# Renatovela-ctrl/dsp-audio-project

Measured on AMD Instinct MI355X. Metric: Msamples/sec SRC→6-biquad EQ→FFT chain at 1/2/4/8 MI355X; % HBM roofline, higher is better.
Workload: dtype f32 (IIR state/coefficients f64); 1 GPU; config 4: 32768 ch x 48000 @48kHz sharded over the GPUs: SRC L3/M2 K121 -> 6-biquad EQ @72kHz -> 4096-pt FFT |X| of centre segment; total_channels=32768, channels_per_gpu=32768, n_in=48000, n_out=72000, fs_in=48000, L=3, M=2, n_fft=4096, parallelism=channel-shard x1 (no collective), launch=hipGraph

## Files before the change

dsp-audio-project_amd/csrc/chain_tile.h:

```cpp
#pragma once
#include <algorithm>
#include <cmath>
#include <cstring>
#include <type_traits>

#include "cascade.h"

namespace dsp {


constexpr int kStream = 2;
constexpr int kSc1 = 16;
constexpr int kLS = 32;
constexpr int kS = 6;
constexpr int kD = 2 * kS;
constexpr int kNPMax = 32;
constexpr int kScanRow = 14;
constexpr int kScanPark = 928;
constexpr int kScanFloats = (kScanPark + 16) * 2;


typedef float f32x4 __attribute__((ext_vector_type(4)));
typedef float f32x2 __attribute__((ext_vector_type(2)));

__host__ __device__ constexpr int xpad(int g) { return g + 4 * (g >> 5); }

template <int L_, int M_, int TT_, int CR_>
struct TileGeo {
  static constexpr int L = L_, M = M_, TT = TT_, CR = CR_;
  static_assert((kLS * L) % M == 0, "32 input samples per sub-chunk must make whole outputs");
  static_assert(M % 2 == 0, "packed taps: windows of one branch share their x parity");
  static constexpr int TSUB = kLS * L / M;
  static constexpr int TILE = kWave * TSUB;
  static_assert(TSUB % 12 == 0 && TSUB <= kWave, "SRC in parts of 12; two float4 halves");
  static constexpr int NP = TT / 2 + 1;
  static_assert(NP <= kNPMax, "tap pairs");
  static constexpr int qi(int i) { return (i * M + CR) / L; }
  static constexpr int phi(int i) { return (i * M + CR) % L; }
  static constexpr int qs(int i) { return qi(i) & ~1; }
  static constexpr int W = qs(TSUB - 1) + 2 * NP;
  static constexpr int NWIN = (kLS * (kWave - 1) + W + 3) / 4 * 4;
  static constexpr int XF = xpad(NWIN + 4) + 4;
  static constexpr int RS = TSUB + 4;
  static constexpr int SF = (kWave / 2) * RS;
  static constexpr int CF = (kWave + 1) * kD * 2;
  static constexpr int LDSF0 = XF > SF ? (XF > CF ? XF : CF) : (SF > CF ? SF : CF);
  static constexpr int LDSF = LDSF0 > kScanFloats ? LDSF0 : kScanFloats;
  static_assert(L <= 4, "four branch slots per tap pair row");
  static_assert(qs(TSUB - 1) < W, "");
};

template <class GEO>
constexpr int branch_parity(int ph) {
  int a = -1;
  for (int i = 0; i < GEO::TSUB; ++i)
    if (GEO::phi(i) == ph) {
      const int ai = GEO::qi(i) & 1;
      if (a >= 0 && a != ai) return -2;
      a = ai;
    }
  return a;
}

constexpr int kGenTS = 32;
constexpr int kGenTile = kWave * kGenTS;
constexpr int kGenWaves = 4;
constexpr int kGenTT = 8;
constexpr int kGenClasses = 8;
constexpr int kGenClassStride = kGenTS * kGenTT + 4;
constexpr int kCtTaps = 10;
constexpr int kCtRow = 12;
constexpr int kCtClassStride = kGenTS * kCtRow + 4;

constexpr int kPpSlots = 16;
constexpr int kPpTapFloats = 1024;

struct TileTables {
  uint64_t key;
  double G[64][kD];
  float Gc[32][kD][2];
  double Q[kD][kD];
  double Dp[6][kS][4];
  double T[kD][kD];
  float TP[kNPMax][4][2];
  int32_t tsub, np, L, M, K, S;
  double cf[kS][4];
  double gain;
  float seq[kGenClasses][kGenTS][kGenTT];
  uint32_t adv[kGenClasses];
  int32_t classes, pad;
  alignas(16) float seqs[kGenClasses][kGenTS][kCtRow];
  float flush_thr;
  int32_t pad3[3];
  alignas(16) float tpw[kPpTapFloats];
  float pp_td;
  int32_t pp_np, pp_geo, pad4;
};

struct TileArgs {
  const float* x;
  float* y;
  float* z;
  const TileTables* tt;
  double* states;
  uint32_t* flags;
  uint32_t* err;
  int64_t B, n_in, ld_x, n_out, ld_y, ntiles, cq;
  int clip;
  uint32_t max_spins;
  const float* taps;
  int64_t c;
  int K, L, M, T, win;
};

__device__ __forceinline__ void fence() { asm volatile("" ::: "memory"); }

__device__ __forceinline__ int lane_id() {
  return (int)__builtin_amdgcn_mbcnt_hi(~0u, __builtin_amdgcn_mbcnt_lo(~0u, 0u));
}

template <int N, class T>
__device__ __forceinline__ void pin(T (&v)[N]) {
#pragma unroll
  for (int i = 0; i < N; ++i) asm volatile("" : "+v"(v[i]));
}

template <class PTR>
__device__ __forceinline__ void mac2(PTR M, double x0, double x1, double& a0, double& a1) {
  a0 = fma(M[0], x0, fma(M[1], x1, a0));
  a1 = fma(M[2], x0, fma(M[3], x1, a1));
}

__device__ __forceinline__ double shfl_up_f64(double v, int d) {
  const int src = ((int)threadIdx.x - d) << 2;
  const uint64_t u = __double_as_longlong(v);
  const uint32_t lo = __builtin_amdgcn_ds_bpermute(src, (int)(uint32_t)u);
  const uint32_t hi = __builtin_amdgcn_ds_bpermute(src, (int)(uint32_t)(u >> 32));
  return __longlong_as_double((long long)(((uint64_t)hi << 32) | lo));
}

__device__ __forceinline__ double shfl_f64(double v, int src) {
  const uint64_t u = __double_as_longlong(v);
  const uint32_t lo = __builtin_amdgcn_ds_bpermute(src << 2, (int)(uint32_t)u);
  const uint32_t hi = __builtin_amdgcn_ds_bpermute(src << 2, (int)(uint32_t)(u >> 32));
  return __longlong_as_double((long long)(((uint64_t)hi << 32) | lo));
}

__device__ __forceinline__ uint32_t load_flag(const uint32_t* p) {
  return __hip_atomic_load((const __attribute__((address_space(1))) uint32_t*)p,
                           __ATOMIC_RELAXED, __HIP_MEMORY_SCOPE_AGENT);
}
__device__ __forceinline__ void store_flag(uint32_t* p, uint32_t v) {
  __hip_atomic_store((__attribute__((address_space(1))) uint32_t*)p, v,
                     __ATOMIC_RELAXED, __HIP_MEMORY_SCOPE_AGENT);
}
__device__ __forceinline__ double load_state(const double* p) {
  return __hip_atomic_load((const __attribute__((address_space(1))) double*)p,
                           __ATOMIC_RELAXED, __HIP_MEMORY_SCOPE_AGENT);
}
__device__ __forceinline__ void store_state(double* p, double v) {
  __hip_atomic_store((__attribute__((address_space(1))) double*)p, v,
                     __ATOMIC_RELAXED, __HIP_MEMORY_SCOPE_AGENT);
}

typedef __attribute__((address_space(4))) const TileTables* tt_ptr;

template <class GEO>
constexpr bool dly_out(int i) { return GEO::phi(i) == 0; }
template <class GEO>
constexpr bool void_pair(int p, int ph) {
  const int a = branch_parity<GEO>(ph);
  if (a < 0) return true;
  for (int e = 0; e < 2; ++e) {
    const int u = 2 * p + e - a;
    if (u >= 0 && u < GEO::TT && ph + GEO::L * (GEO::TT - 1 - u) < 40 * GEO::L + 1) return false;
  }
  return true;
}
struct VoidPairs {
  bool v[kNPMax][4];
};
template <class GEO>
constexpr VoidPairs void_pairs() {
  VoidPairs t{};
  for (int p = 0; p < kNPMax; ++p)
    for (int ph = 0; ph < 4; ++ph) t.v[p][ph] = ph < GEO::L && p < GEO::NP && void_pair<GEO>(p, ph);
  return t;
}
template <class GEO>
constexpr int dly_slot() { return GEO::TT / 2 + (branch_parity<GEO>(0) > 0 ? 1 : 0); }

template <class GEO, int H0, int NH, bool DLY = false>
__device__ __forceinline__ void src_part(const float* xw, tt_ptr tt, float (&y)[GEO::TSUB]) {
  static constexpr VoidPairs kVoid = void_pairs<GEO>();
  constexpr int V0 = GEO::qs(H0) / 4 * 4;
  constexpr int V1 = GEO::qs(H0 + NH - 1) + 2 * GEO::NP;
  constexpr int NV = (V1 - V0 + 3) / 4 * 4;
  f32x2 w[NV / 2];
#pragma unroll
  for (int k = 0; k < NV / 4; ++k) {
    const f32x4 f = *reinterpret_cast<const f32x4*>(xw + xpad(V0 + 4 * k));
    w[2 * k] = f32x2{f.x, f.y};
    w[2 * k + 1] = f32x2{f.z, f.w};
  }
  f32x2 acc[NH];
#pragma unroll
  for (int i = 0; i < NH; ++i) acc[i] = f32x2{0.f, 0.f};
#pragma unroll
  for (int p = 0; p < GEO::NP; ++p) {
    tt_ptr tq = tt;
    asm volatile("" : "+s"(tq));
    f32x2 t[GEO::L];
#pragma unroll
    for (int ph = 0; ph < GEO::L; ++ph) t[ph] = f32x2{tq->TP[p][ph][0], tq->TP[p][ph][1]};
#pragma unroll
    for (int i = 0; i < NH; ++i)
      if (!(DLY && (dly_out<GEO>(H0 + i) || kVoid.v[p][GEO::phi(H0 + i)])))
        acc[i] = __builtin_elementwise_fma(t[GEO::phi(H0 + i)],
                                           w[(GEO::qs(H0 + i) - V0) / 2 + p], acc[i]);
  }
  float td = 0.f;
  if (DLY) {
    tt_ptr tq = tt;
    asm volatile("" : "+s"(tq));
    td = tq->TP[dly_slot<GEO>() / 2][0][dly_slot<GEO>() % 2];
  }
#pragma unroll
  for (int i = 0; i < NH; ++i) {
    if (DLY && dly_out<GEO>(H0 + i)) {
      const f32x2 xv = w[(GEO::qs(H0 + i) - V0) / 2 + dly_slot<GEO>() / 2];
      y[H0 + i] = td * (dly_slot<GEO>() % 2 ? xv.y : xv.x);
    } else {
      y[H0 + i] = acc[i].x + acc[i].y;
    }
  }
}

template <int TS>
struct StageBase {
  int b[3];
  __device__ __forceinline__ explicit StageBase(int lane) {
    if constexpr (TS == 32) {
      b[0] = 32 * (lane >> 3) + 4 * ((lane & 7) ^ ((lane >> 3) & 7));
    } else if constexpr (TS != 48) {
      static_assert(TS % 4 == 0, "staging rows of whole float4s");
      b[0] = lane;
    } else {
      const int a = (lane * 43) >> 9;
      const int r = lane - 12 * a;
      b[0] = 4 * lane + 4 * a;
      b[1] = b[0] + 4 * ((r + 8) >> 4);
      b[2] = b[0] + 4 * ((r + 12) >> 4);
    }
  }
  __device__ __forceinline__ int at(int k) const {
    if constexpr (TS == 32) return b[0] + 256 * k;
    else if constexpr (TS != 48) {
      const int g = 4 * (b[0] + kWave * k);
      return g + 4 * (g / TS);
    } else return b[k % 3] + 276 * k + (k >= 3 ? 4 : 0);
  }
};

template <int TS>
__device__ __forceinline__ void store_tile(float* lds, const float (&v)[TS], int lane,
                                           __amdgpu_buffer_rsrc_t rs) {
  constexpr int RS = TS == 32 ? 32 : TS + 4;
  constexpr int NF4 = (kWave / 2) * TS / 4;
  constexpr int NR = (NF4 + kWave - 1) / kWave;
  typedef unsigned int u32x4 __attribute__((ext_vector_type(4)));
  const StageBase<TS> sb(lane);
#pragma unroll
  for (int h = 0; h < 2; ++h) {
    fence();
    if ((lane >> 5) == h) {
      float* row = lds + (lane & 31) * RS;
      const int sw = TS == 32 ? (lane & 7) : 0;
#pragma unroll
      for (int k = 0; k < TS / 4; ++k)
        *reinterpret_cast<float4*>(row + 4 * (k ^ sw)) =
            make_float4(v[4 * k], v[4 * k + 1], v[4 * k + 2], v[4 * k + 3]);
    }
    fence();
#pragma unroll
    for (int k = 0; k < NR; ++k) {
      const int g = 4 * (lane + kWave * k);
      const bool past = NF4 % kWave && k == NR - 1 && lane + kWave * k >= NF4;
      const float4 f = *reinterpret_cast<const float4*>(lds + sb.at(k));
      u32x4 d;
      d.x = __float_as_uint(f.x);
      d.y = __float_as_uint(f.y);
      d.z = __float_as_uint(f.z);
      d.w = __float_as_uint(f.w);
      __builtin_amdgcn_raw_buffer_store_b128(d, rs, past ? 0x7ffffff0 : (h * (kWave / 2) * TS + g) * 4,
                                             0, kStream);
    }
  }
  fence();
}

__device__ __forceinline__ void tile_entry_state(const TileArgs& a, int64_t b, int64_t tile,
                                                 int lane, double (&m_in)[kD]) {
  if (lane == 0) {
    const int64_t prev = b * a.ntiles + tile - 1;
    uint32_t spins = 0;
    bool ok = true;
    while (load_flag(a.flags + prev) == 0u) {
      if (++spins > a.max_spins) {
        store_flag(a.err, 1u);
        ok = false;
        break;
      }
      __builtin_amdgcn_s_sleep(2);
    }
    fence();
#pragma unroll
    for (int d = 0; d < kD; ++d) m_in[d] = load_state(a.states + prev * kD + d);
    if (ok) store_flag(a.flags + prev, 0u);
  }
}

__host__ __device__ constexpr int staging_floats(int ts) { return (kWave / 2) * (ts + 4); }

__device__ __forceinline__ void pass1_basis(tt_ptr mt, const f32x2 (&e2)[kD], double (&v)[kD]);

template <int TS>
__device__ __forceinline__ void pass1_state(tt_ptr mt, const float (&y)[TS], double (&v)[kD]) {
  {
    f32x2 e2[kD];
#pragma unroll
    for (int d = 0; d < kD; ++d) e2[d] = f32x2{-0.f, -0.f};
#pragma unroll
    for (int j = 0; j < TS / 2; ++j) {
      tt_ptr tq = mt;
      asm volatile("" : "+s"(tq));
      const f32x2 u = f32x2{y[2 * j], y[2 * j + 1]};
#pragma unroll
      for (int d = 0; d < kD; ++d)
        e2[d] = __builtin_elementwise_fma(f32x2{tq->Gc[j][d][0], tq->Gc[j][d][1]}, u, e2[d]);
    }
    pin(e2);
    pass1_basis(mt, e2, v);
  }
}

template <int TS>
__device__ __forceinline__ void pass1_state_f64(tt_ptr mt, const float (&y)[TS], double (&v)[kD]) {
#pragma unroll
  for (int d = 0; d < kD; ++d) v[d] = 0.0;
#pragma unroll
  for (int i = 0; i < TS; ++i) {
    tt_ptr tq = mt;
    asm volatile("" : "+s"(tq));
    const double u = (double)y[i];
#pragma unroll
    for (int d = 0; d < kD; ++d) v[d] = fma(tq->G[i][d], u, v[d]);
  }
}

__device__ __forceinline__ void pass1_basis(tt_ptr mt, const f32x2 (&e2)[kD], double (&v)[kD]) {
  {
    f32x2 e[kS];
#pragma unroll
    for (int k = 0; k < kS; ++k)
      e[k] = f32x2{e2[2 * k].x + e2[2 * k].y, e2[2 * k + 1].x + e2[2 * k + 1].y};
    double ed[kD];
#pragma unroll
    for (int k = 0; k < kS; ++k) {
      ed[2 * k] = (double)e[k].x;
      ed[2 * k + 1] = (double)e[k].y;
    }
#pragma unroll
    for (int r = kD - 1; r >= 0; --r) {
      tt_ptr tq = mt;
      asm volatile("" : "+s"(tq));
      double acc = tq->Q[r][0] * ed[0];
#pragma unroll
      for (int c = 1; c <= r; ++c) acc = fma(tq->Q[r][c], ed[c], acc);
      v[r] = acc;
    }
  }
}

template <int TS, bool NANCLIP>
__device__ __forceinline__ void pass2_cascade(const TileArgs& a, tt_ptr mt, float (&y)[TS],
                                              const double (&m)[kD]) {
  double s1[kS], s2[kS];
#pragma unroll
  for (int r = 0; r < kD; ++r) {
    double acc = m[r];
#pragma unroll
    for (int cc = 0; cc < (r / 2) * 2; ++cc) acc = fma(mt->T[r][cc], m[cc], acc);
    if (r & 1) s2[r / 2] = acc;
    else s1[r / 2] = acc;
  }
  float lo = a.clip ? -1.f : -INFINITY, hi = a.clip ? 1.f : INFINITY;
  asm volatile("" : "+v"(lo), "+v"(hi));
  const float g32 = (float)mt->gain;
  {
    double pend[kS];
#pragma unroll
    for (int st = 0; st < TS + kS - 1; ++st) {
#pragma unroll
      for (int k = kS - 1; k >= 0; --k) {
        const int t = st - k;
        if (t < 0 || t >= TS) continue;
        const double u = k == 0 ? (double)y[t] : pend[k - 1];
        const double c1 = mt->cf[k][0], c2 = mt->cf[k][1], a1 = mt->cf[k][2], a2 = mt->cf[k][3];
        const double w = fma(-a2, s2[k], fma(-a1, s1[k], u));
        const double v2 = fma(c2, s2[k], fma(c1, s1[k], w));
        s2[k] = s1[k];
        s1[k] = w;
        if (k == kS - 1)
          y[t] = NANCLIP ? clip_f32((float)v2 * g32, lo, hi)
                         : __builtin_amdgcn_fmed3f((float)v2 * g32, lo, hi);
        else pend[k] = v2;
      }
    }
  }
}

template <int TS, bool P1F64 = false, class SUMS>
__device__ __forceinline__ void fix_outputs(const TileArgs& a, tt_ptr mt, int64_t b, int64_t z0,
                                            float (&y)[TS], double (&v)[kD], SUMS&& sums) {
  const __amdgpu_buffer_rsrc_t rz = __builtin_amdgcn_make_buffer_rsrc(
      a.z + b * a.ld_y, 0, (int)(a.n_out * 4), 0x00020000);
  const int off0 = (int)(z0 * 4);
  auto get = [&](int i) {
    return __uint_as_float(__builtin_amdgcn_raw_buffer_load_b32(rz, off0 + 4 * i, 0, 1));
  };
  auto put = [&](int i, float f) {
    __builtin_amdgcn_raw_buffer_store_b32(__float_as_uint(f), rz, off0 + 4 * i, 0, 0);
  };
#pragma unroll
  for (int i = 0; i < TS; ++i) put(i, y[i]);
  asm volatile("s_waitcnt vmcnt(0)" ::: "memory");
  bool any = false;
#pragma unroll 1
  for (int i = 0; i < TS; ++i) {
    float nf, fin, f = get(i);
    sums(i, nf, fin);
    any |= nf_fix(f, nf, fin);
    put(i, f);
  }
  asm volatile("s_waitcnt vmcnt(0)" ::: "memory");
  if (any) {
#pragma unroll
    for (int d = 0; d < kD; ++d) v[d] = __builtin_nan("");
  } else if constexpr (P1F64) {
#pragma unroll
    for (int d = 0; d < kD; ++d) v[d] = 0.0;
#pragma unroll 1
    for (int i = 0; i < TS; ++i) {
      const double u = (double)get(i);
#pragma unroll
      for (int d = 0; d < kD; ++d) v[d] = fma(mt->G[i][d], u, v[d]);
    }
  } else {
    f32x2 e2[kD];
#pragma unroll
    for (int d = 0; d < kD; ++d) e2[d] = f32x2{0.f, 0.f};
#pragma unroll 1
    for (int j = 0; j < TS / 2; ++j) {
      const f32x2 u = f32x2{get(2 * j), get(2 * j + 1)};
#pragma unroll
      for (int d = 0; d < kD; ++d)
        e2[d] = __builtin_elementwise_fma(f32x2{mt->Gc[j][d][0], mt->Gc[j][d][1]}, u, e2[d]);
    }
    pass1_basis(mt, e2, v);
  }
#pragma unroll
  for (int i = 0; i < TS; ++i) y[i] = get(i);
}

struct ChainedEntry {};
struct RegCarry {
  double c0, c1;
};
struct EarlyEntry {
  bool early;
  const double* slot;
};
struct AggEntry {};
struct GivenEntry {};

template <int TS, bool YST = true, bool REPAIR = false, bool P1F64 = false, class ONNF,
          class ENTRY = ChainedEntry>
__device__ __forceinline__ void tile_cascade(const TileArgs& a, tt_ptr mt, float* lds,
                                             float (&y)[TS], int lane, int64_t b, int64_t tile,
                                             int64_t m0, ONNF&& on_nf, ENTRY&& entry = ENTRY{}) {
  constexpr bool kRegCarry = std::is_same_v<std::decay_t<ENTRY>, RegCarry>;
  constexpr bool kEarly = std::is_same_v<std::decay_t<ENTRY>, EarlyEntry>;
  constexpr bool kAgg = std::is_same_v<std::decay_t<ENTRY>, AggEntry>;
  constexpr bool kGiven = std::is_same_v<std::decay_t<ENTRY>, GivenEntry>;
  double v[kD];
  if constexpr (P1F64) pass1_state_f64<TS>(mt, y, v);
  else pass1_state<TS>(mt, y, v);
  if constexpr (REPAIR) {
    if (__builtin_amdgcn_ballot_w64(!__builtin_isfinite(v[kD - 1]))) on_nf(y, v);
  }
  pin(v);

  typedef double f64x2 __attribute__((ext_vector_type(2)));
  double* rows = reinterpret_cast<double*>(lds);
  double* park = rows + kScanPark;
  static_assert(kScanPark >= 65 * kScanRow, "park row past the scan rows");
#pragma unroll
  for (int k = 0; k < kS; ++k)
    *reinterpret_cast<f64x2*>(rows + lane * kScanRow + 2 * k) = f64x2{v[2 * k], v[2 * k + 1]};
  if constexpr (kGiven) {
    if (lane == 0) {
      const int64_t me = b * a.ntiles + tile;
#pragma unroll
      for (int k = 0; k < kS; ++k)
        *reinterpret_cast<f64x2*>(park + 2 * k) =
            *reinterpret_cast<const f64x2*>(a.states + me * kD + 2 * k);
    }
  } else if (kAgg || tile == 0) {
    if (lane == 0) {
#pragma unroll
      for (int k = 0; k < kS; ++k) *reinterpret_cast<f64x2*>(park + 2 * k) = f64x2{0.0, 0.0};
    }
  } else if constexpr (kRegCarry) {
    if ((lane >> 3) == 7)
      *reinterpret_cast<f64x2*>(park + 2 * (lane & 7)) = f64x2{entry.c0, entry.c1};
  } else {
    bool got = false;
    if constexpr (kEarly) {
      if (entry.early) {
        asm volatile("s_waitcnt vmcnt(0)" ::: "memory");
        if (lane == 0) {
#pragma unroll
          for (int k = 0; k < kS; ++k)
            *reinterpret_cast<f64x2*>(park + 2 * k) =
                *reinterpret_cast<const f64x2*>(entry.slot + 2 * k);
          store_flag(a.flags + b * a.ntiles + tile - 1, 0u);
        }
        got = true;
      }
    }
    if (!got) {
      double m_in[kD];
      tile_entry_state(a, b, tile, lane, m_in);
      if (lane == 0) {
#pragma unroll
        for (int d = 0; d < kD; ++d) park[d] = m_in[d];
      }
    }
  }
  fence();
  const int sg = lane >> 3;
  const bool worker = (lane & 7) < 6;
  const int kb = lane & 7;
  const __attribute__((address_space(1))) double* Dg =
      (const __attribute__((address_space(1))) double*)&mt->Dp[0][kb][0];
  const f64x2 d0a = *reinterpret_cast<const __attribute__((address_space(1))) f64x2*>(Dg);
  const f64x2 d0b = *reinterpret_cast<const __attribute__((address_space(1))) f64x2*>(Dg + 2);
  f64x2 e[8];
#pragma unroll
  for (int i = 0; i < 8; ++i)
    e[i] = *reinterpret_cast<const f64x2*>(rows + (8 * sg + i) * kScanRow + 2 * kb);
  const __attribute__((address_space(1))) double* D8g = Dg + 3 * kS * 4;
  f64x2 p8a = *reinterpret_cast<const __attribute__((address_space(1))) f64x2*>(D8g);
  f64x2 p8b = *reinterpret_cast<const __attribute__((address_space(1))) f64x2*>(D8g + 2);
  double u0 = e[0].x, u1 = e[0].y;
#pragma unroll
  for (int i = 1; i < 8; ++i) {
    const double n0 = fma(d0a.x, u0, fma(d0a.y, u1, e[i].x));
    const double n1 = fma(d0b.x, u0, fma(d0b.y, u1, e[i].y));
    u0 = n0;
    u1 = n1;
  }
  f64x2 mi = f64x2{0.0, 0.0};
  if (sg == 0) {
    mi = *reinterpret_cast<const f64x2*>(park + 2 * kb);
    u0 = fma(p8a.x, mi.x, fma(p8a.y, mi.y, u0));
    u1 = fma(p8b.x, mi.x, fma(p8b.y, mi.y, u1));
  }
#pragma unroll
  for (int lv = 0; lv < 3; ++lv) {
    const int dd = 1 << lv;
    const int ss = sg - dd;
    const int src = ss >= 0 ? lane - 8 * dd : lane;
    const double x0 = shfl_f64(u0, src), x1 = shfl_f64(u1, src);
    if (ss >= 0) {
      u0 = fma(p8a.x, x0, fma(p8a.y, x1, u0));
      u1 = fma(p8b.x, x0, fma(p8b.y, x1, u1));
    }
    if (lv < 2) {
      const f64x2 qa = f64x2{fma(p8a.x, p8a.x, p8a.y * p8b.x), fma(p8a.x, p8a.y, p8a.y * p8b.y)};
      const f64x2 qb = f64x2{fma(p8b.x, p8a.x, p8b.y * p8b.x), fma(p8b.x, p8a.y, p8b.y * p8b.y)};
      p8a = qa;
      p8b = qb;
    }
  }
  {
    const int ss = sg - 1;
    const int src = ss >= 0 ? lane - 8 : lane;
    const double x0 = shfl_f64(u0, src), x1 = shfl_f64(u1, src);
    u0 = ss >= 0 ? x0 : mi.x;
    u1 = ss >= 0 ? x1 : mi.y;
  }
  f64x2* const wr = reinterpret_cast<f64x2*>(rows + (8 * sg + 1) * kScanRow) + (kb < 6 ? kb : 6);
#pragma unroll
  for (int i = 0; i < 8; ++i) {
    const double n0 = fma(d0a.x, u0, fma(d0a.y, u1, e[i].x));
    const double n1 = fma(d0b.x, u0, fma(d0b.y, u1, e[i].y));
    u0 = n0;
    u1 = n1;
    wr[i * (kScanRow / 2)] = f64x2{u0, u1};
  }
  static_assert(kScanRow == 14, "six blocks and one padding slot per scan row");
  {
    const int64_t me = b * a.ntiles + tile;
    if (worker && sg == 7) {
      store_state(a.states + me * kD + 2 * kb, u0);
      store_state(a.states + me * kD + 2 * kb + 1, u1);
    }
    if constexpr (kRegCarry) {
      entry.c0 = u0;
      entry.c1 = u1;
    }
  }
  if constexpr (kAgg) return;
  const bool raise = !kRegCarry && !kGiven && tile + 1 < a.ntiles;
  auto raise_flag = [&] {
    if (lane == 8 * 7) store_flag(a.flags + b * a.ntiles + tile, 1u);
  };
  fence();
  double m[kD];
  {
    const double* src = lane == 0 ? park : rows + lane * kScanRow;
#pragma unroll
    for (int k = 0; k < kS; ++k) {
      const f64x2 t = *reinterpret_cast<const f64x2*>(src + 2 * k);
      m[2 * k] = t.x;
      m[2 * k + 1] = t.y;
    }
  }
  fence();

  if (YST && a.y) {
    const __amdgpu_buffer_rsrc_t ry = __builtin_amdgcn_make_buffer_rsrc(
        a.y + b * a.ld_y + m0, 0, (int)((a.n_out - m0) * 4), 0x00020000);
    store_tile<TS>(lds, y, lane, ry);
    if (raise) {
      asm volatile("s_waitcnt vmcnt(%0)" ::"n"(TS / 4) : "memory");
      raise_flag();
    }
  } else if (raise) {
    asm volatile("s_waitcnt vmcnt(0)" ::: "memory");
    raise_flag();
  }
  pin(y);
  pass2_cascade<TS, REPAIR>(a, mt, y, m);
  const __amdgpu_buffer_rsrc_t rz = __builtin_amdgcn_make_buffer_rsrc(
      a.z + b * a.ld_y + m0, 0, (int)((a.n_out - m0) * 4), 0x00020000);
  int lane_z = lane;
  asm volatile("" : "+v"(lane_z));
  store_tile<TS>(lds, y, lane_z, rz);
}

template <class BODY>
__device__ __forceinline__ void repair_channel(const TileArgs& a, int lane, int64_t b,
                                               BODY&& body) {
  const double* st = a.states + b * a.ntiles * kD + (kD - 1);
  uint32_t* fl = a.flags + b * a.ntiles;
  int64_t first = a.ntiles;
  for (int64_t t0 = 0; t0 < a.ntiles && first == a.ntiles; t0 += kWave) {
    const int64_t t = t0 + lane;
    const uint64_t bad =
        __builtin_amdgcn_ballot_w64(t < a.ntiles && !__builtin_isfinite(st[t * kD]));
    if (bad) first = t0 + __builtin_ctzll(bad);
  }
  for (int64_t tile = first; tile < a.ntiles; ++tile) {
    if (lane == 0 && tile > 0) store_flag(fl + tile - 1, 1u);
    asm volatile("s_waitcnt vmcnt(0)" ::: "memory");
    body(tile);
    asm volatile("s_waitcnt vmcnt(0)" ::: "memory");
    if (lane == 0) store_flag(fl + tile, 0u);
  }
}

template <class BODY>
__device__ __forceinline__ void repair_channels(const TileArgs& a, int wave, int waves,
                                                BODY&& body) {
  const int lane = lane_id();
  const int64_t stride = (int64_t)gridDim.x * waves * kWave;
  for (int64_t b0 = ((int64_t)blockIdx.x * waves + wave) * kWave; b0 < a.B; b0 += stride) {
    const int64_t b = b0 + lane;
    const double last = b < a.B ? a.states[(b * a.ntiles + a.ntiles - 1) * kD + (kD - 1)] : 0.0;
    uint64_t bad = __builtin_amdgcn_ballot_w64(!__builtin_isfinite(last));
    while (bad) {
      const int64_t bb = b0 + __builtin_ctzll(bad);
      bad &= bad - 1;
      repair_channel(a, lane, bb, [&](int64_t tile) { body(bb, tile); });
    }
  }
}

}
```

dsp-audio-project_amd/csrc/chain_tile.hip:

```cpp
#include <algorithm>
#include <cmath>
#include <cstring>
#include <type_traits>

#include "cascade.h"

#include "chain_pp.h"
#include "chain_tile.h"

namespace dsp {
namespace {

template <class GEO, bool DLY, bool REPAIR, int MODE = 0>
__device__ __forceinline__ void chain_tile_body(const TileArgs& a, float* lds, int lane, int64_t b,
                                                int64_t tile) {
  constexpr int TS = GEO::TSUB;
  const int64_t m0 = tile * GEO::TILE;
  const tt_ptr mt = (tt_ptr)a.tt;

  uint32_t fl = 0;
  if (!REPAIR && MODE == 0 && tile > 0 && lane == 0)
    fl = load_flag(a.flags + b * a.ntiles + tile - 1);

  {
    const __amdgpu_buffer_rsrc_t rx = __builtin_amdgcn_make_buffer_rsrc(
        const_cast<float*>(a.x) + b * a.ld_x, 0, (int)(a.n_in * 4), 0x00020000);
    const int64_t xs0 = m0 * GEO::M / GEO::L + a.cq - (GEO::TT - 1);
    constexpr int NF = GEO::NWIN / 4;
    const int off0 = (int)(xs0 * 4) + 16 * lane;
    float* const l0 = lds + 4 * lane + 4 * (lane >> 3);
#pragma unroll
    for (int k = 0; k < (NF + kWave - 1) / kWave; ++k) {
      if ((k + 1) * kWave <= NF || lane + kWave * k < NF) {
        const f32x4 v = __builtin_amdgcn_raw_buffer_load_b128(rx, off0 + 1024 * k, 0, kStream);
        *reinterpret_cast<f32x4*>(l0 + 288 * k) = v;
      }
    }
    static_assert(xpad(4 * (kWave + 7)) - xpad(4 * 7) == 288, "xpad: 288 floats per 64 float4s");
  }
  fence();
  EarlyEntry early{false, reinterpret_cast<const double*>(lds + GEO::LDSF)};
  if (!REPAIR && MODE == 0 && tile > 0 && __builtin_amdgcn_readfirstlane(fl) == 1u) {
    early.early = true;
    if (lane < 2 * kD) {
      const int64_t prev = b * a.ntiles + tile - 1;
      __builtin_amdgcn_global_load_lds(
          (const __attribute__((address_space(1))) void*)(reinterpret_cast<const uint32_t*>(
                                                               a.states + prev * kD) + lane),
          (__attribute__((address_space(3))) void*)(lds + GEO::LDSF), 4, 0, kSc1);
    }
  }

  float y[TS];
  {
    const float* xw = lds + 36 * lane;
    static_assert(TS == 48, "SRC parts of 48 / 24 outputs");
    if constexpr (DLY) {
      src_part<GEO, 0, 48, true>(xw, mt, y);
      pin(y);
    } else {
      src_part<GEO, 0, 24, false>(xw, mt, y);
      pin(y);
      src_part<GEO, 24, 24, false>(xw, mt, y);
      pin(y);
    }
  }
  if constexpr (REPAIR) {
    auto fix = [&](float (&yy)[TS], double (&v)[kD]) {
      const float thr = mt->flush_thr;
      fix_outputs(a, mt, b, m0 + TS * lane, yy, v, [&](int i, float& nf, float& fin) {
        const int j = i * GEO::M + GEO::CR;
        const int base = kLS * lane + j / GEO::L + GEO::TT - 1;
        window_sums(a.taps, a.K, GEO::L, j % GEO::L, thr, base,
                    [&](int t) { return lds[xpad(base - t)]; }, nf, fin);
      });
    };
    tile_cascade<TS, true, true>(a, mt, lds, y, lane, b, tile, m0, fix);
  } else if constexpr (MODE == 1) {
    tile_cascade<TS>(a, mt, lds, y, lane, b, tile, m0, 0, AggEntry{});
  } else if constexpr (MODE == 2) {
    tile_cascade<TS>(a, mt, lds, y, lane, b, tile, m0, 0, GivenEntry{});
  } else {
    tile_cascade<TS>(a, mt, lds, y, lane, b, tile, m0, 0, early);
  }
}

template <class GEO, bool DLY = false>
__global__ __launch_bounds__(kWave) __attribute__((amdgpu_waves_per_eu(4))) void k_chain_tile(
    TileArgs a) {
  __shared__ __attribute__((aligned(16))) float lds[GEO::LDSF + 2 * kD];
  const int64_t tile = blockIdx.y, b = blockIdx.x;
  chain_tile_body<GEO, DLY, false>(a, lds, threadIdx.x, b, tile);
}

template <class GEO, bool DLY, int MODE>
__global__ __launch_bounds__(kWave) __attribute__((amdgpu_waves_per_eu(4))) void k_chain_tile3(
    TileArgs a) {
  __shared__ __attribute__((aligned(16))) float lds[GEO::LDSF];
  chain_tile_body<GEO, DLY, false, MODE>(a, lds, threadIdx.x, blockIdx.x, blockIdx.y);
}

template <class GEO, bool DLY = false>
__global__ __launch_bounds__(kWave) void k_chain_tile_repair(TileArgs a) {
  __shared__ __attribute__((aligned(16))) float lds[GEO::LDSF + 2 * kD];
  repair_channels(a, 0, 1, [&](int64_t b, int64_t tile) {
    chain_tile_body<GEO, DLY, true>(a, lds, (int)threadIdx.x, b, tile);
  });
}

__device__ __forceinline__ int gen_wave() {
  return __builtin_amdgcn_readfirstlane((int)(threadIdx.x / kWave));
}

__device__ __forceinline__ void gen_load_window(const TileArgs& a, float* win, int lane, int64_t b,
                                                int64_t qa) {
  const __amdgpu_buffer_rsrc_t rx = __builtin_amdgcn_make_buffer_rsrc(
      const_cast<float*>(a.x) + b * a.ld_x, 0, (int)(a.n_in * 4), 0x00020000);
  const int nf = a.win >> 2;
  for (int f0 = 0; f0 < nf; f0 += 8 * kWave) {
    f32x4 v[8];
#pragma unroll
    for (int r = 0; r < 8; ++r) {
      const int f = f0 + r * kWave + lane;
      v[r] = __builtin_amdgcn_raw_buffer_load_b128(rx, (int)((qa + 4 * f) * 4), 0, kStream);
    }
#pragma unroll
    for (int r = 0; r < 8; ++r) {
      const int f = f0 + r * kWave + lane;
      if (f < nf) *reinterpret_cast<f32x4*>(win + 4 * f) = v[r];
    }
  }
}

__device__ __forceinline__ void gen_load_classes(const TileArgs& a, float* seq, uint32_t* adv) {
  constexpr int kNT = kWave * kGenWaves;
  constexpr int kF4 = kGenTS * kGenTT / 4;
  const int C = ((tt_ptr)a.tt)->classes;
  const f32x4* src = reinterpret_cast<const f32x4*>(a.tt->seq);
  f32x4 v[2];
#pragma unroll
  for (int r = 0; r < 2; ++r) v[r] = src[(r * kNT + threadIdx.x) & (kGenClasses * kF4 - 1)];
#pragma unroll
  for (int r = 0; r < 2; ++r) {
    const int i = r * kNT + threadIdx.x, k = i / kF4, f = i - k * kF4;
    if (k < C) *reinterpret_cast<f32x4*>(seq + k * kGenClassStride + 4 * f) = v[r];
  }
  if (threadIdx.x < kGenClasses) adv[threadIdx.x] = a.tt->adv[threadIdx.x];
  __syncthreads();
}

__device__ __forceinline__ void gen_fix(const TileArgs& a, tt_ptr mt, const float* win, int64_t qa,
                                        int64_t j0, int64_t b, int64_t z0, float (&yy)[kGenTS],
                                        double (&v)[kD]) {
  const float thr = mt->flush_thr;
  fix_outputs(a, mt, b, z0, yy, v, [&](int i, float& nf, float& fin) {
    const int64_t j = j0 + (int64_t)i * a.M, q = j / a.L;
    const int base = (int)(q - qa);
    window_sums(a.taps, a.K, a.L, (int)(j - q * a.L), thr, a.T - 1,
                [&](int t) { return win[base - t]; }, nf, fin);
  });
}

template <bool UP, bool REPAIR, class ENTRY = ChainedEntry>
__device__ __forceinline__ void chain_gen_body(const TileArgs& a, const float* seq,
                                               const uint32_t* adv, float* win, int lane,
                                               int64_t b, int64_t tile, ENTRY&& entry = ENTRY{}) {
  const int L = a.L, M = a.M, T = a.T;
  const tt_ptr mt = (tt_ptr)a.tt;
  const int C = mt->classes;
  const int64_t m0 = tile * kGenTile;

  const int64_t qlo = (m0 * M + a.c) / L - (T - 1);
  const int64_t qa = (qlo >> 2) << 2;
  gen_load_window(a, win, lane, b, qa);
  fence();

  float y[kGenTS];
  const int64_t j0 = (m0 + (int64_t)kGenTS * lane) * M + a.c;
  {
    const int jl = (int)(m0 * M + a.c) + kGenTS * M * lane;
    int qr = jl / L - (T - 1) - (int)qa;
    const int dq = M / L;
    const int cls = ((int)tile * kWave + lane) % C;
    const float* row = seq + cls * kGenClassStride;
    const uint32_t am = adv[cls];
    float w[kGenTT];
#pragma unroll
    for (int u = 0; u < kGenTT; ++u) w[u] = win[qr + u];
    float4 h0 = *reinterpret_cast<const float4*>(row);
    float4 h1 = *reinterpret_cast<const float4*>(row + 4);
    float nx = UP ? win[qr + kGenTT] : 0.f;
#pragma unroll
    for (int i = 0; i < kGenTS; ++i) {
      const bool carry = (am >> i) & 1u;
      const int qr_n = qr + dq + (carry ? 1 : 0);
      float4 h0n, h1n;
      float nxn = 0.f, wn[kGenTT];
      if (i + 1 < kGenTS) {
        h0n = *reinterpret_cast<const float4*>(row + kGenTT * (i + 1));
        h1n = *reinterpret_cast<const float4*>(row + kGenTT * (i + 1) + 4);
        if constexpr (UP) {
          nxn = win[qr_n + kGenTT];
        } else {
#pragma unroll
          for (int u = 0; u < kGenTT; ++u) wn[u] = win[qr_n + u];
        }
      }
      f32x2 acc = {0.f, 0.f};
      acc = __builtin_elementwise_fma(f32x2{h0.x, h0.y}, f32x2{w[0], w[1]}, acc);
      acc = __builtin_elementwise_fma(f32x2{h0.z, h0.w}, f32x2{w[2], w[3]}, acc);
      acc = __builtin_elementwise_fma(f32x2{h1.x, h1.y}, f32x2{w[4], w[5]}, acc);
      acc = __builtin_elementwise_fma(f32x2{h1.z, h1.w}, f32x2{w[6], w[7]}, acc);
      y[i] = acc.x + acc.y;
      if (i + 1 < kGenTS) {
        if constexpr (UP) {
#pragma unroll
          for (int u = 0; u < kGenTT - 1; ++u) w[u] = carry ? w[u + 1] : w[u];
          w[kGenTT - 1] = carry ? nx : w[kGenTT - 1];
          nx = nxn;
        } else {
#pragma unroll
          for (int u = 0; u < kGenTT; ++u) w[u] = wn[u];
        }
        h0 = h0n;
        h1 = h1n;
        qr = qr_n;
      }
    }
  }
  pin(y);
  if constexpr (REPAIR)
    tile_cascade<kGenTS, true, true>(a, mt, win, y, lane, b, tile, m0,
                                     [&](float (&yy)[kGenTS], double (&v)[kD]) {
                                       gen_fix(a, mt, win, qa, j0, b, m0 + kGenTS * lane, yy, v);
                                     });
  else
    tile_cascade<kGenTS>(a, mt, win, y, lane, b, tile, m0, 0, entry);
}

template <bool UP>
__global__ __launch_bounds__(kWave * kGenWaves) __attribute__((amdgpu_waves_per_eu(4))) void
k_chain_gen(TileArgs a) {
  extern __shared__ __attribute__((aligned(16))) float smem[];
  const int w = gen_wave();
  const int lane = threadIdx.x & (kWave - 1);
// ... 828 lines not shown
  if (B < 1 || !tile_geometry(n_in, n_out, K, L, M, c, S, &tp)) return 0;
  if (tp.kind == 4) {
    const PpEntry& e = kPpEntries[tp.pp];
    const bool ident = e.LR == 1 && e.MR == 1 && e.NP == 1 && e.UC == 0;
    if (three_launch(B, tp.ntiles, ident ? kTileCostIdent : kTileCostSrc)) return 3;
  }
  if (tp.kind != 4 && three_launch(B, tp.ntiles, kTileCostSrc)) return 3;
  return 1;
}

size_t chain_tile_workspace_bytes(int64_t B, int64_t n_in, int64_t n_out, int K, int L, int M,
                                  int64_t c, int S) {
  TilePlan tp;
  if (B <= 0 || !tile_geometry(n_in, n_out, K, L, M, c, S, &tp)) return 256;
  return tile_ws(B, tp.ntiles).total;
}

size_t chain_tile_tables_bytes() { return sizeof(TileTables); }

int chain_tile_tables(void* out, size_t out_bytes, int64_t n_in, int64_t n_out, const float* taps,
                      int K, int L, int M, int64_t c, const double* sos, int S, uint64_t* key) {
  if (key) *key = 0;
  TilePlan tp;
  if (!tile_geometry(n_in, n_out, K, L, M, c, S, &tp)) return kNotFused;
  DSP_REQUIRE(out && out_bytes >= sizeof(TileTables), "tables buffer too small: %zu < %zu bytes",
              out_bytes, sizeof(TileTables));
  DSP_REQUIRE(taps && (S == 0 || sos), "null pointer");
  SosParams p;
  if (S > 0 && !realize(sos, S, &p)) return kNotFused;
  if (S == 0) realize(nullptr, 0, &p);
  TileTables* tt = static_cast<TileTables*>(out);
  std::memset(tt, 0, sizeof(TileTables));
  if (!modal_tables(p, S, (int)tp.tsub, tt)) return kNotFused;
  std::vector<float> ft(taps, taps + K);
  const float thr = tap_flush_threshold(taps, K, L);
  for (float& t : ft) t = flush_tap(t, thr);
  tt->flush_thr = thr;
  bool dly = false;
  if (tp.kind == 1) {
    tap_pairs<Geo3241>(ft.data(), K, tt);
    dly = delay_branch<Geo3241>(tt);
  } else if (tp.kind == 4) {
    if (!pp_rows(ft.data(), K, L, M, c, kPpEntries[tp.pp], tt)) return kNotFused;
    tt->pp_geo = tp.pp;
  } else {
    gen_sequences(ft.data(), K, L, M, c, tt);
  }
  if (tp.kind == 3) ct_sequences(ft.data(), K, L, M, c, tt);
  for (int k = 0; k < kS; ++k) {
    tt->cf[k][0] = p.c[k][1];
    tt->cf[k][1] = p.c[k][2];
    tt->cf[k][2] = p.c[k][3];
    tt->cf[k][3] = p.c[k][4];
  }
  tt->gain = p.G;
  for (int r = 0; r < kD; ++r)
    for (int c = 0; c < kD; ++c) tt->Q[r][c] /= p.G;
  for (int i = 0; i < 64; ++i)
    for (int c = 0; c < kD; ++c) tt->G[i][c] /= p.G;
  tt->tsub = (int32_t)tp.tsub;
  tt->np = tp.kind == 1 ? Geo3241::NP : 0;
  tt->L = L;
  tt->M = M;
  tt->K = K;
  tt->S = S;
  tt->key = dly ? dly_key(tables_key(tp, n_in, n_out, K, L, M, c, sos, S))
                : tables_key(tp, n_in, n_out, K, L, M, c, sos, S);
  if (key) *key = tt->key;
  return DSP_OK;
}

int launch_chain_tile(const float* x, float* y, float* z, int64_t B, int64_t n_in, int64_t ld_x,
                      int64_t n_out, int64_t ld_y, const float* taps, int K, int L, int M,
                      int64_t c, const double* sos, int S, int clip, const void* tables,
                      uint64_t key, uint32_t max_spins, int variant, void* ws, size_t ws_bytes,
                      hipStream_t s) {
  TilePlan tp;
  if (!tables || !tile_geometry(n_in, n_out, K, L, M, c, S, &tp)) return kNotFused;
  DSP_REQUIRE(taps, "null taps");
  const uint64_t key0 = tables_key(tp, n_in, n_out, K, L, M, c, sos, S);
  const bool dly = key == dly_key(key0);
  if (key != key0 && !dly) return kNotFused;
  auto aligned = [B](const void* p, int64_t ld) {
    return (B == 1 || (ld & 3) == 0) && (reinterpret_cast<uintptr_t>(p) & 15) == 0;
  };
  if (!aligned(x, ld_x) || (y && !aligned(y, ld_y)) || !aligned(z, ld_y)) return kNotFused;
  SosParams p;
  if (S > 0 && !realize(sos, S, &p)) return kNotFused;
  if (S == 0) realize(nullptr, 0, &p);
  const TileWs w = tile_ws(B, tp.ntiles);
  DSP_REQUIRE(ws && ws_bytes >= w.total, "chain workspace too small: %zu < %zu bytes", ws_bytes,
              w.total);
  DSP_REQUIRE((reinterpret_cast<uintptr_t>(ws) & 255) == 0, "chain workspace not 256-B aligned");
  DSP_REQUIRE((reinterpret_cast<uintptr_t>(tables) & 255) == 0, "chain tables not 256-B aligned");
  DSP_REQUIRE(B * tp.ntiles < ((int64_t)1 << 31), "batch too large for one launch");
  char* base = static_cast<char*>(ws);
  TileArgs a;
  a.x = x;
  a.y = y;
  a.z = z;
  a.tt = static_cast<const TileTables*>(tables);
  a.states = reinterpret_cast<double*>(base + w.st_off);
  a.flags = reinterpret_cast<uint32_t*>(base + w.fl_off);
  a.err = reinterpret_cast<uint32_t*>(base + w.err_off);
  a.B = B;
  a.n_in = n_in;
  a.ld_x = ld_x;
  a.n_out = n_out;
  a.ld_y = ld_y;
  a.ntiles = tp.ntiles;
  a.cq = c / L;
  a.clip = clip;
  a.max_spins = max_spins;
  a.taps = taps;
  a.c = c;
  a.K = K;
  a.L = L;
  a.M = M;
  a.T = (K + L - 1) / L;
  a.win = tp.win;
  const bool one_wave = tp.kind == 1 || tp.kind == 4;
  const int64_t groups = one_wave ? B : ceil_div(B, (int64_t)kGenWaves);
  const int64_t rwaves = one_wave ? 1 : kGenWaves;
  const unsigned rgrid =
      (unsigned)std::min<int64_t>(ceil_div(B, kWave * rwaves), kRepairGroups);
  if (tp.kind == 4) {
    const PpNeed n = pp_need(K, L, M, c);
    a.cq = n.xa0;
    const PpEntry& e = kPpEntries[tp.pp];
    const bool ident = e.LR == 1 && e.MR == 1 && e.NP == 1 && e.UC == 0;
    const bool three = variant != 2 &&
        (variant == 4 || three_launch(B, tp.ntiles, ident ? kTileCostIdent : kTileCostSrc));
    int rc = launch_chain_pp_0(e, a, rgrid, three, s);
    if (rc == kNotFused) rc = launch_chain_pp_1(e, a, rgrid, three, s);
    if (rc == kNotFused) rc = launch_chain_pp_2(e, a, rgrid, three, s);
    if (rc == kNotFused) rc = launch_chain_pp_3(e, a, rgrid, three, s);
    if (rc == kNotFused) return set_error(DSP_EINVAL, "no per-phase kernel for entry %d", tp.pp);
    return rc;
  } else if (tp.kind == 1) {
    const dim3 grid((unsigned)B, (unsigned)tp.ntiles);
    if (variant != 2 && (variant == 4 || three_launch(B, tp.ntiles, kTileCostSrc))) {
      {
        TraceScope trace("chain_tile_agg", s);
        auto k1 = dly ? k_chain_tile3<Geo3241, true, 1> : k_chain_tile3<Geo3241, false, 1>;
        hipLaunchKernelGGL(k1, grid, dim3(kWave), 0, s, a);
      }
      launch_tile_carry(a, Geo3241::TSUB, s);
      TraceScope trace("chain_tile", s);
      auto k3 = dly ? k_chain_tile3<Geo3241, true, 2> : k_chain_tile3<Geo3241, false, 2>;
      hipLaunchKernelGGL(k3, grid, dim3(kWave), 0, s, a);
    } else {
      TraceScope trace("chain_tile", s);
      auto kern = dly ? k_chain_tile<Geo3241, true> : k_chain_tile<Geo3241, false>;
      hipLaunchKernelGGL(kern, grid, dim3(kWave), 0, s, a);
    }
    TraceScope trace("chain_repair", s);
    auto rep = dly ? k_chain_tile_repair<Geo3241, true> : k_chain_tile_repair<Geo3241, false>;
    hipLaunchKernelGGL(rep, dim3(rgrid), dim3(kWave), 0, s, a);
  } else if (tp.kind == 3) {
    DSP_REQUIRE(groups * tp.ntiles < ((int64_t)1 << 31), "batch too large for one launch");
    const size_t shm = ct_lds_bytes(gen_classes(L, M), tp.win);
    auto kern = a.T <= 7 ? k_chain_gct<160, 147, true> : k_chain_gct<160, 147, false>;
    auto rep = a.T <= 7 ? k_chain_gct_repair<160, 147, true> : k_chain_gct_repair<160, 147, false>;
    auto pers = a.T <= 7 ? k_chain_gcp<160, 147, true> : k_chain_gcp<160, 147, false>;
    if (int rc = allow_lds(kern, shm)) return rc;
    if (int rc = allow_lds(rep, shm)) return rc;
    if (int rc = allow_lds(pers, shm)) return rc;
    const int res = a.T <= 7 ? resident_groups<k_chain_gcp<160, 147, true>>(kWave * kGenWaves, shm)
                             : resident_groups<k_chain_gcp<160, 147, false>>(kWave * kGenWaves, shm);
    const int64_t rounds = res > 0 ? ceil_div(groups, res) : 0;
    const bool fits = tp.win <= 4 * kGcpWin * kWave && tp.win > 4 * (kGcpWin - 1) * kWave;
    const bool three = variant == 4 || (variant == 0 && three_launch(B, tp.ntiles, kTileCostSrc));
    const bool persistent = !three && fits && res > 0 && groups >= res &&
                            groups * 8 >= rounds * res * 7 && variant != 2;
    if (three) {
      auto k1 = a.T <= 7 ? k_chain_gct3<160, 147, true, 1> : k_chain_gct3<160, 147, false, 1>;
      auto k3 = a.T <= 7 ? k_chain_gct3<160, 147, true, 2> : k_chain_gct3<160, 147, false, 2>;
      if (int rc = allow_lds(k1, shm)) return rc;
      if (int rc = allow_lds(k3, shm)) return rc;
      {
        TraceScope trace("chain_tile_agg", s);
        hipLaunchKernelGGL(k1, dim3((unsigned)groups, (unsigned)tp.ntiles), dim3(kWave * kGenWaves),
                           shm, s, a);
      }
      launch_tile_carry(a, kGenTS, s);
      TraceScope trace("chain_tile", s);
      hipLaunchKernelGGL(k3, dim3((unsigned)groups, (unsigned)tp.ntiles), dim3(kWave * kGenWaves),
                         shm, s, a);
    } else {
      TraceScope trace("chain_tile", s);
      if (persistent || (variant == 3 && fits))
        hipLaunchKernelGGL(pers, dim3((unsigned)std::min<int64_t>(groups, std::max(res, 1))),
                           dim3(kWave * kGenWaves), shm, s, a);
      else
        hipLaunchKernelGGL(kern, dim3((unsigned)groups, (unsigned)tp.ntiles), dim3(kWave * kGenWaves),
                           shm, s, a);
    }
    TraceScope trace("chain_repair", s);
    hipLaunchKernelGGL(rep, dim3(rgrid), dim3(kWave * kGenWaves), shm, s, a);
  } else {
    DSP_REQUIRE(groups * tp.ntiles < ((int64_t)1 << 31), "batch too large for one launch");
    const size_t shm = gen_lds_bytes(tp.win);
    auto kern = M < L ? k_chain_gen<true> : k_chain_gen<false>;
    auto rep = M < L ? k_chain_gen_repair<true> : k_chain_gen_repair<false>;
    if (int rc = allow_lds(kern, shm)) return rc;
    if (int rc = allow_lds(rep, shm)) return rc;
    const dim3 grid((unsigned)groups, (unsigned)tp.ntiles);
    if (variant != 2 && (variant == 4 || three_launch(B, tp.ntiles, kTileCostSrc))) {
      auto k1 = M < L ? k_chain_gen3<true, 1> : k_chain_gen3<false, 1>;
      auto k3 = M < L ? k_chain_gen3<true, 2> : k_chain_gen3<false, 2>;
      if (int rc = allow_lds(k1, shm)) return rc;
      if (int rc = allow_lds(k3, shm)) return rc;
      {
        TraceScope trace("chain_tile_agg", s);
        hipLaunchKernelGGL(k1, grid, dim3(kWave * kGenWaves), shm, s, a);
      }
      launch_tile_carry(a, kGenTS, s);
      TraceScope trace("chain_tile", s);
      hipLaunchKernelGGL(k3, grid, dim3(kWave * kGenWaves), shm, s, a);
    } else {
      TraceScope trace("chain_tile", s);
      hipLaunchKernelGGL(kern, grid, dim3(kWave * kGenWaves), shm, s, a);
    }
    TraceScope trace("chain_repair", s);
    hipLaunchKernelGGL(rep, dim3(rgrid), dim3(kWave * kGenWaves), shm, s, a);
  }
  DSP_LAUNCHED("k_chain_tile");
  return DSP_OK;
}

}
```

Before: 275,400 Msamples/s.

## Pack two channels' short last tiles into one wave via pair kernel

```diff
diff --git a/dsp-audio-project_amd/csrc/chain_tile.h b/dsp-audio-project_amd/csrc/chain_tile.h
--- a/dsp-audio-project_amd/csrc/chain_tile.h
+++ b/dsp-audio-project_amd/csrc/chain_tile.h
@@ -18,6 +18,8 @@
 constexpr int kScanRow = 14;
 constexpr int kScanPark = 928;
 constexpr int kScanFloats = (kScanPark + 16) * 2;
+constexpr int kScanPark2 = 16;
+constexpr int kScanFloatsPair = (kScanPark + 2 * kScanPark2) * 2;
 
 
 typedef float f32x4 __attribute__((ext_vector_type(4)));
@@ -262,9 +264,10 @@
   }
 };
 
-template <int TS>
-__device__ __forceinline__ void store_tile(float* lds, const float (&v)[TS], int lane,
-                                           __amdgpu_buffer_rsrc_t rs) {
+template <int TS, bool PAIR>
+__device__ __forceinline__ void store_tile_rs(float* lds, const float (&v)[TS], int lane,
+                                              __amdgpu_buffer_rsrc_t rs,
+                                              __amdgpu_buffer_rsrc_t rs1) {
   constexpr int RS = TS == 32 ? 32 : TS + 4;
   constexpr int NF4 = (kWave / 2) * TS / 4;
   constexpr int NR = (NF4 + kWave - 1) / kWave;
@@ -292,11 +295,18 @@
       d.y = __float_as_uint(f.y);
       d.z = __float_as_uint(f.z);
       d.w = __float_as_uint(f.w);
-      __builtin_amdgcn_raw_buffer_store_b128(d, rs, past ? 0x7ffffff0 : (h * (kWave / 2) * TS + g) * 4,
-                                             0, kStream);
+      __builtin_amdgcn_raw_buffer_store_b128(
+          d, PAIR && h ? rs1 : rs,
+          past ? 0x7ffffff0 : ((PAIR ? 0 : h * (kWave / 2) * TS) + g) * 4, 0, kStream);
     }
   }
   fence();
+}
+
+template <int TS>
+__device__ __forceinline__ void store_tile(float* lds, const float (&v)[TS], int lane,
+                                           __amdgpu_buffer_rsrc_t rs) {
+  store_tile_rs<TS, false>(lds, v, lane, rs, rs);
 }
 
 __device__ __forceinline__ void tile_entry_state(const TileArgs& a, int64_t b, int64_t tile,
@@ -483,6 +493,12 @@
 };
 struct AggEntry {};
 struct GivenEntry {};
+struct PairEntry {
+  bool early[2];
+  const double* slot;
+  int64_t b2;
+  bool has2;
+};
 
 template <int TS, bool YST = true, bool REPAIR = false, bool P1F64 = false, class ONNF,
           class ENTRY = ChainedEntry>
@@ -493,6 +509,15 @@
   constexpr bool kEarly = std::is_same_v<std::decay_t<ENTRY>, EarlyEntry>;
   constexpr bool kAgg = std::is_same_v<std::decay_t<ENTRY>, AggEntry>;
   constexpr bool kGiven = std::is_same_v<std::decay_t<ENTRY>, GivenEntry>;
+  constexpr bool kPair = std::is_same_v<std::decay_t<ENTRY>, PairEntry>;
+  int hf = 0;
+  int64_t bh = b;
+  bool live = true;
+  if constexpr (kPair) {
+    hf = lane >> 5;
+    bh = hf ? entry.b2 : b;
+    live = !hf || entry.has2;
+  }
   double v[kD];
   if constexpr (P1F64) pass1_state_f64<TS>(mt, y, v);
   else pass1_state<TS>(mt, y, v);
@@ -515,6 +540,32 @@
       for (int k = 0; k < kS; ++k)
         *reinterpret_cast<f64x2*>(park + 2 * k) =
             *reinterpret_cast<const f64x2*>(a.states + me * kD + 2 * k);
+    }
+  } else if constexpr (kPair) {
+    const bool leader = (lane & 31) == 0;
+    double* const pk = park + kScanPark2 * hf;
+    const bool mine = tile > 0 && (hf ? entry.early[1] : entry.early[0]);
+    if (tile > 0 && (entry.early[0] || entry.early[1]))
+      asm volatile("s_waitcnt vmcnt(0)" ::: "memory");
+    if (leader && mine) {
+#pragma unroll
+      for (int k = 0; k < kS; ++k)
+        *reinterpret_cast<f64x2*>(pk + 2 * k) =
+            *reinterpret_cast<const f64x2*>(entry.slot + 16 * hf + 2 * k);
+      store_flag(a.flags + bh * a.ntiles + tile - 1, 0u);
+    }
+    const bool wait = tile > 0 && leader && live && !mine;
+    if (__builtin_amdgcn_ballot_w64(wait)) {
+      double m_in[kD];
+      tile_entry_state(a, bh, tile, wait ? 0 : 1, m_in);
+      if (wait) {
+#pragma unroll
+        for (int d = 0; d < kD; ++d) pk[d] = m_in[d];
+      }
+    }
+    if (leader && !mine && !wait) {
+#pragma unroll
+      for (int k = 0; k < kS; ++k) *reinterpret_cast<f64x2*>(pk + 2 * k) = f64x2{0.0, 0.0};
     }
   } else if (kAgg || tile == 0) {
     if (lane == 0) {
@@ -550,6 +601,8 @@
   }
   fence();
   const int sg = lane >> 3;
+  constexpr int kSegs = kPair ? 4 : 8, kLevels = kPair ? 2 : 3;
+  const int sq = kPair ? (sg & 3) : sg;
   const bool worker = (lane & 7) < 6;
   const int kb = lane & 7;
   const __attribute__((address_space(1))) double* Dg =
@@ -572,22 +625,22 @@
     u1 = n1;
   }
   f64x2 mi = f64x2{0.0, 0.0};
-  if (sg == 0) {
-    mi = *reinterpret_cast<const f64x2*>(park + 2 * kb);
+  if (sq == 0) {
+    mi = *reinterpret_cast<const f64x2*>(park + kScanPark2 * hf + 2 * kb);
     u0 = fma(p8a.x, mi.x, fma(p8a.y, mi.y, u0));
     u1 = fma(p8b.x, mi.x, fma(p8b.y, mi.y, u1));
   }
 #pragma unroll
-  for (int lv = 0; lv < 3; ++lv) {
+  for (int lv = 0; lv < kLevels; ++lv) {
     const int dd = 1 << lv;
-    const int ss = sg - dd;
+    const int ss = sq - dd;
     const int src = ss >= 0 ? lane - 8 * dd : lane;
     const double x0 = shfl_f64(u0, src), x1 = shfl_f64(u1, src);
     if (ss >= 0) {
       u0 = fma(p8a.x, x0, fma(p8a.y, x1, u0));
       u1 = fma(p8b.x, x0, fma(p8b.y, x1, u1));
     }
-    if (lv < 2) {
+    if (lv < kLevels - 1) {
       const f64x2 qa = f64x2{fma(p8a.x, p8a.x, p8a.y * p8b.x), fma(p8a.x, p8a.y, p8a.y * p8b.y)};
       const f64x2 qb = f64x2{fma(p8b.x, p8a.x, p8b.y * p8b.x), fma(p8b.x, p8a.y, p8b.y * p8b.y)};
       p8a = qa;
@@ -595,7 +648,7 @@
     }
   }
   {
-    const int ss = sg - 1;
+    const int ss = sq - 1;
     const int src = ss >= 0 ? lane - 8 : lane;
     const double x0 = shfl_f64(u0, src), x1 = shfl_f64(u1, src);
     u0 = ss >= 0 ? x0 : mi.x;
@@ -612,8 +665,8 @@
   }
   static_assert(kScanRow == 14, "six blocks and one padding slot per scan row");
   {
-    const int64_t me = b * a.ntiles + tile;
-    if (worker && sg == 7) {
+    const int64_t me = bh * a.ntiles + tile;
+    if (worker && sq == kSegs - 1 && live) {
       store_state(a.states + me * kD + 2 * kb, u0);
       store_state(a.states + me * kD + 2 * kb + 1, u1);
     }
@@ -623,14 +676,15 @@
     }
   }
   if constexpr (kAgg) return;
-  const bool raise = !kRegCarry && !kGiven && tile + 1 < a.ntiles;
+  const bool raise = !kRegCarry && !kGiven && !kPair && tile + 1 < a.ntiles;
   auto raise_flag = [&] {
     if (lane == 8 * 7) store_flag(a.flags + b * a.ntiles + tile, 1u);
   };
   fence();
   double m[kD];
   {
-    const double* src = lane == 0 ? park : rows + lane * kScanRow;
+    const double* src = (kPair ? (lane & 31) == 0 : lane == 0) ? park + kScanPark2 * hf
+                                                               : rows + lane * kScanRow;
 #pragma unroll
     for (int k = 0; k < kS; ++k) {
       const f64x2 t = *reinterpret_cast<const f64x2*>(src + 2 * k);
@@ -640,10 +694,20 @@
   }
   fence();
 
+  auto store = [&](float* p, const __amdgpu_buffer_rsrc_t rs, int ln) {
+    if constexpr (kPair) {
+      const __amdgpu_buffer_rsrc_t rs1 = __builtin_amdgcn_make_buffer_rsrc(
+          p + (entry.has2 ? entry.b2 : b) * a.ld_y + m0, 0,
+          entry.has2 ? (int)((a.n_out - m0) * 4) : 0, 0x00020000);
+      store_tile_rs<TS, true>(lds, y, ln, rs, rs1);
+    } else {
+      store_tile<TS>(lds, y, ln, rs);
+    }
+  };
   if (YST && a.y) {
     const __amdgpu_buffer_rsrc_t ry = __builtin_amdgcn_make_buffer_rsrc(
         a.y + b * a.ld_y + m0, 0, (int)((a.n_out - m0) * 4), 0x00020000);
-    store_tile<TS>(lds, y, lane, ry);
+    store(a.y, ry, lane);
     if (raise) {
       asm volatile("s_waitcnt vmcnt(%0)" ::"n"(TS / 4) : "memory");
       raise_flag();
@@ -658,7 +722,7 @@
       a.z + b * a.ld_y + m0, 0, (int)((a.n_out - m0) * 4), 0x00020000);
   int lane_z = lane;
   asm volatile("" : "+v"(lane_z));
-  store_tile<TS>(lds, y, lane_z, rz);
+  store(a.z, rz, lane_z);
 }
 
 template <class BODY>
diff --git a/dsp-audio-project_amd/csrc/chain_tile.hip b/dsp-audio-project_amd/csrc/chain_tile.hip
--- a/dsp-audio-project_amd/csrc/chain_tile.hip
+++ b/dsp-audio-project_amd/csrc/chain_tile.hip
@@ -91,6 +91,97 @@
   __shared__ __attribute__((aligned(16))) float lds[GEO::LDSF + 2 * kD];
   const int64_t tile = blockIdx.y, b = blockIdx.x;
   chain_tile_body<GEO, DLY, false>(a, lds, threadIdx.x, b, tile);
+}
+
+template <class GEO>
+struct PairGeo {
+  static constexpr int XB = (kLS * (kWave / 2 - 1) + GEO::W + 31) / 32 * 32;
+  static_assert(xpad(XB + kLS) - xpad(XB) == 36, "half 1's lane windows 36 floats apart");
+  static constexpr int NWIN = (XB + kLS * (kWave / 2 - 1) + GEO::W + 3) / 4 * 4;
+  static constexpr int XF = xpad(NWIN + 4) + 4;
+  static constexpr int LDSF0 = XF > GEO::LDSF ? XF : GEO::LDSF;
+  static constexpr int LDSF = LDSF0 > kScanFloatsPair ? LDSF0 : kScanFloatsPair;
+  static constexpr int SLOT = kWave;
+};
+
+template <class GEO, bool DLY>
+__device__ __forceinline__ void chain_tile_pair_body(const TileArgs& a, float* lds, int lane,
+                                                     int64_t b, int64_t b2, bool has2) {
+  typedef PairGeo<GEO> PG;
+  constexpr int TS = GEO::TSUB;
+  const int64_t tile = a.ntiles - 1;
+  const int64_t m0 = tile * GEO::TILE;
+  const tt_ptr mt = (tt_ptr)a.tt;
+  const int hf = lane >> 5;
+  const int64_t bx = has2 ? b2 : b;
+
+  uint32_t fl = 0;
+  if (tile > 0 && (lane & 31) == 0 && (!hf || has2))
+    fl = load_flag(a.flags + (hf ? b2 : b) * a.ntiles + tile - 1);
+
+  {
+    const __amdgpu_buffer_rsrc_t rx0 = __builtin_amdgcn_make_buffer_rsrc(
+        const_cast<float*>(a.x) + b * a.ld_x, 0, (int)(a.n_in * 4), 0x00020000);
+    const __amdgpu_buffer_rsrc_t rx1 = __builtin_amdgcn_make_buffer_rsrc(
+        const_cast<float*>(a.x) + bx * a.ld_x, 0, has2 ? (int)(a.n_in * 4) : 0, 0x00020000);
+    const int64_t xs0 = m0 * GEO::M / GEO::L + a.cq - (GEO::TT - 1);
+    constexpr int NF = PG::NWIN / 4, NA = PG::XB / 4;
+    const int off0 = (int)(xs0 * 4) + 16 * lane;
+    float* const l0 = lds + 4 * lane + 4 * (lane >> 3);
+#pragma unroll
+    for (int k = 0; k < (NF + kWave - 1) / kWave; ++k) {
+      const int f = lane + kWave * k;
+      if (k * kWave < NA && ((k + 1) * kWave <= NA || f < NA)) {
+        const f32x4 v = __builtin_amdgcn_raw_buffer_load_b128(rx0, off0 + 1024 * k, 0, kStream);
+        *reinterpret_cast<f32x4*>(l0 + 288 * k) = v;
+      }
+      if ((k + 1) * kWave > NA && (k * kWave >= NA || f >= NA) &&
+          ((k + 1) * kWave <= NF || f < NF)) {
+        const f32x4 v = __builtin_amdgcn_raw_buffer_load_b128(rx1, off0 + 1024 * k - 4 * PG::XB, 0,
+                                                              kStream);
+        *reinterpret_cast<f32x4*>(l0 + 288 * k) = v;
+      }
+    }
+  }
+  fence();
+  PairEntry entry{{false, false}, reinterpret_cast<const double*>(lds + PG::LDSF), b2, has2};
+  if (tile > 0) {
+    entry.early[0] = __builtin_amdgcn_readlane(fl, 0) == 1u;
+    entry.early[1] = __builtin_amdgcn_readlane(fl, 32) == 1u;
+    if (entry.early[0] || entry.early[1]) {
+      const int64_t prev = (hf ? bx : b) * a.ntiles + tile - 1;
+      const int j = lane & 31;
+      __builtin_amdgcn_global_load_lds(
+          (const __attribute__((address_space(1))) void*)(reinterpret_cast<const uint32_t*>(
+                                                               a.states + prev * kD) +
+                                                           (j < 2 * kD ? j : j - 2 * kD)),
+          (__attribute__((address_space(3))) void*)(lds + PG::LDSF), 4, 0, kSc1);
+    }
+  }
+
+  float y[TS];
+  {
+    const float* xw = lds + 36 * lane + hf * (xpad(PG::XB) - 36 * (kWave / 2));
+    static_assert(TS == 48, "SRC parts of 48 / 24 outputs");
+    if constexpr (DLY) {
+      src_part<GEO, 0, 48, true>(xw, mt, y);
+      pin(y);
+    } else {
+      src_part<GEO, 0, 24, false>(xw, mt, y);
+      pin(y);
+      src_part<GEO, 24, 24, false>(xw, mt, y);
+      pin(y);
+    }
+  }
+  tile_cascade<TS>(a, mt, lds, y, lane, b, tile, m0, 0, entry);
+}
+
+template <class GEO, bool DLY = false>
+__global__ __launch_bounds__(kWave) __attribute__((amdgpu_waves_per_eu(4))) void
+k_chain_tile_pair(TileArgs a) {
+  __shared__ __attribute__((aligned(16))) float lds[PairGeo<GEO>::LDSF + PairGeo<GEO>::SLOT];
+  const int64_t b = 2 * (int64_t)blockIdx.x;
+  chain_tile_pair_body<GEO, DLY>(a, lds, threadIdx.x, b, b + 1, b + 1 < a.B);
 }
 
 template <class GEO, bool DLY, int MODE>
@@ -1225,7 +1316,16 @@
     } else {
       TraceScope trace("chain_tile", s);
       auto kern = dly ? k_chain_tile<Geo3241, true> : k_chain_tile<Geo3241, false>;
-      hipLaunchKernelGGL(kern, grid, dim3(kWave), 0, s, a);
+      const int64_t tail = n_out - (tp.ntiles - 1) * Geo3241::TILE;
+      if (B >= 2 && ceil_div(tail, (int64_t)Geo3241::TSUB) <= kWave / 2) {
+        if (tp.ntiles > 1)
+          hipLaunchKernelGGL(kern, dim3((unsigned)B, (unsigned)(tp.ntiles - 1)), dim3(kWave), 0, s,
+                             a);
+        auto pair = dly ? k_chain_tile_pair<Geo3241, true> : k_chain_tile_pair<Geo3241, false>;
+        hipLaunchKernelGGL(pair, dim3((unsigned)ceil_div(B, 2)), dim3(kWave), 0, s, a);
+      } else {
+        hipLaunchKernelGGL(kern, grid, dim3(kWave), 0, s, a);
+      }
     }
     TraceScope trace("chain_repair", s);
     auto rep = dly ? k_chain_tile_repair<Geo3241, true> : k_chain_tile_repair<Geo3241, false>;
```

Measured after the change: 278,500 Msamples/s (median of 6 runs). 1.01x the previous value.
